# Project-MONAI/MONAI

Measured on AMD Instinct MI355X. Metric: voxels/s sliding-window 3D seg (512^3 vol, 96^3 win, ov 0.5) at 1/8 GPU, higher is better.
Workload: dtype f32; 1 GPU; BasicUNet 5-class seed 1, 512^3 CT phantom in HBM, 96^3 win ov 0.5 gaussian, sw_batch 4 (engine: <= 64 windows per launch); parallelism=1 GPU

## Files before the change

### monai_amd/csrc/kernels/conv3d_wino_h2.h

```cpp
#pragma once
#include "common.h"
#include "conv3d_h2.h"

namespace mh {

constexpr int HWG_BY = 4, HWG_BX = 16;
constexpr int HWG_RY = HWG_BY + 2, HWG_RX = HWG_BX + 2;
constexpr int HWG_NP = HWG_RY * HWG_RX;
constexpr int HWG_PB = 144;
constexpr int HWG_DB = (HWG_NP + 1) * HWG_PB;
constexpr int HWG_ZB = 32 * 1024;
constexpr int HWG_OPS = 24;
constexpr int HWG_CIN = 32, HWG_CN = 32;
constexpr int HWG_WAVES = 8;
constexpr unsigned HWG_DROP = 0x80000000u;

__device__ __forceinline__ void hw_split4(const f32x4 v, u32x2& hi, u32x2& lo) {
    _Float16 h_[4], l_[4];
#pragma unroll
    for (int i = 0; i < 4; ++i) {
        h_[i] = (_Float16)v[i];
        float r = v[i] - (float)h_[i];
        MH_OPAQUE(r);
        l_[i] = (_Float16)r;
    }
    const f16x2 h01 = {h_[0], h_[1]}, h23 = {h_[2], h_[3]}, l01 = {l_[0], l_[1]}, l23 = {l_[2], l_[3]};
    hi = u32x2{__builtin_bit_cast(unsigned, h01), __builtin_bit_cast(unsigned, h23)};
    lo = u32x2{__builtin_bit_cast(unsigned, l01), __builtin_bit_cast(unsigned, l23)};
}

__device__ __forceinline__ f32x4 hw_fma4(const f32x4 a, const float s, const f32x4 c) { return __builtin_elementwise_fma(a, f32x4{s, s, s, s}, c); }
__device__ __forceinline__ void hw_split4p(const f32x4 v, const float m1, u32x2& hi, u32x2& lo) {
#ifdef MH_SIMT_EMULATOR
    f16x2 h01, l01, h23, l23;
    h2_split_pair(v[0], v[1], m1, h01, l01);
    h2_split_pair(v[2], v[3], m1, h23, l23);
    hi = u32x2{__builtin_bit_cast(unsigned, h01), __builtin_bit_cast(unsigned, h23)};
    lo = u32x2{__builtin_bit_cast(unsigned, l01), __builtin_bit_cast(unsigned, l23)};
#else
    unsigned h0, h1, l0, l1;
    asm("v_cvt_pk_f16_f32 %0, %1, %2" : "=v"(h0) : "v"(v[0]), "v"(v[1]));
    asm("v_cvt_pk_f16_f32 %0, %1, %2" : "=v"(h1) : "v"(v[2]), "v"(v[3]));
    asm("v_fma_mixlo_f16 %0, %1, %2, %3 op_sel_hi:[1,0,0]" : "=v"(l0) : "v"(h0), "v"(m1), "v"(v[0]));
    asm("v_fma_mixlo_f16 %0, %1, %2, %3 op_sel_hi:[1,0,0]" : "=v"(l1) : "v"(h1), "v"(m1), "v"(v[2]));
    asm("v_fma_mixhi_f16 %0, %1, %2, %3 op_sel:[1,0,0] op_sel_hi:[1,0,0]" : "+v"(l0) : "v"(h0), "v"(m1), "v"(v[1]));
    asm("v_fma_mixhi_f16 %0, %1, %2, %3 op_sel:[1,0,0] op_sel_hi:[1,0,0]" : "+v"(l1) : "v"(h1), "v"(m1), "v"(v[3]));
    hi = u32x2{h0, h1};
    lo = u32x2{l0, l1};
#endif
}
__device__ __forceinline__ float hw_xchg32(const float x, const int hi) {
#ifdef MH_SIMT_EMULATOR
    (void)hi;
    return __shfl_xor(x, 32);
#else
    const auto r = __builtin_amdgcn_permlane32_swap(__builtin_bit_cast(unsigned, x), __builtin_bit_cast(unsigned, x), false, false);
    return __builtin_bit_cast(float, hi ? r[0] : r[1]);
#endif
}
#ifdef MH_SIMT_EMULATOR
#define MH_HW_KEEP_BRANCH ((void)0)
#else
#define MH_HW_KEEP_BRANCH asm volatile("" ::: "memory")
#endif

struct HwFinish {
    int co_l, fa, g4, frp, fq;
};
__device__ __forceinline__ HwFinish hw_finish_role(const int wave, const int lane) {
    HwFinish r;
    r.fq = lane & 3;
    r.frp = r.fq & 1;
    r.fa = lane >> 5;
    r.g4 = ((wave >> 1) & 1) ? (r.fq >> 1 ? 2 : 1) : (r.fq >> 1 ? 3 : 0);
    r.co_l = (wave >> 2) * 16 + (wave & 1) * 8 + ((lane >> 2) & 7);
    return r;
}

template <bool STATS, bool ACC = false, bool POOL = false>
__global__ void __launch_bounds__(512)
conv3d_k3_h2w_kernel(Tensor in, const uint4* __restrict__ wp, const float* __restrict__ wtail, const float* __restrict__ bias, Tensor out,
                     float* __restrict__ stats, int bxn, int byn, int zchunk, unsigned nblk, float* __restrict__ pmax, float* __restrict__ pmin,
                     long long pool_n_stride) {
    __shared__ __attribute__((aligned(16))) char smem[3 * HWG_DB + 2 * HWG_ZB];
    __shared__ unsigned bound_s[4];
    char* const ds = smem;
    char* const zs_ = smem + 3 * HWG_DB;
    const int tid = threadIdx.x, lane = tid & 63;
    const int wave = __builtin_amdgcn_readfirstlane(tid >> 6);
    const int wi = wave & 3, jp = wave >> 2;
    const int Cout = out.C, D = out.D, H = out.H, W = out.W;
    const long long HW = (long long)H * W, DHW = (long long)D * HW;

    const unsigned ncg = (unsigned)(Cout / HWG_CN);
    unsigned lid = xcd_remap(blockIdx.x, gridDim.x);
    const int cg = (int)(lid % ncg);
    lid /= ncg;
    const unsigned b = lid % nblk;
    const int n = (int)(lid / nblk);
    const int x0 = (int)(b % bxn) * HWG_BX, y0 = (int)((b / bxn) % byn) * HWG_BY;
    const int zs = (int)(b / (bxn * byn)) * zchunk, ze = min(zs + zchunk, D);
    const int p_first = max(zs - 1, 0), p_last = min(ze, D - 1);

    unsigned soff;
    int loff[2];
    {
        const int pr = min(lane, 53);
        const int ly = pr / 9;
        int lx = 2 * (pr - 9 * ly);
        const int gy = y0 + ly - 1;
        int gx = x0 + lx - 1;
        if (gx < 0) { gx += 1; lx += 1; }
        if (gx + 1 >= W) { gx -= 1; lx -= 1; }
        const bool ok = lane < 54 && gy >= 0 && gy < H;
        soff = ok ? 4u * (unsigned)(gy * W + gx) : 0u;
        loff[0] = (ok ? ly * HWG_RX + lx : HWG_NP) * HWG_PB;
        loff[1] = (ok ? ly * HWG_RX + lx + 1 : HWG_NP) * HWG_PB;
    }
    for (int i = tid; i < (3 * HWG_DB + 2 * HWG_ZB) / 16; i += 512) reinterpret_cast<uint4*>(smem)[i] = make_uint4(0u, 0u, 0u, 0u);
    f32x4 nra, nrb, nrs;
    {
        unsigned mb = 0u;
        if (lane < HWG_CIN) {
            const float4 a = *reinterpret_cast<const float4*>(in.nrm + (long long)n * in.nrm_n_stride + 4LL * lane);
            const unsigned bb = abs_bits(a.w);
            mb = bb == 0u ? 0x7fc00000u : bb;
        }
        mb = wave_umax(mb);
        if (tid == 0) bound_s[0] = mb;
    }
    __syncthreads();
    int e_in = 0;
    bool poisoned = false;
    {
        const unsigned mb = bound_s[0];
        poisoned = mb >= 0x7f800000u;
        e_in = poisoned ? 0 : min(max(13 - ((int)(mb >> 23) - 126), -100), 100);
        const float p_ = __uint_as_float((unsigned)(e_in + 127) << 23);
#pragma unroll
        for (int i = 0; i < 4; ++i) {
            const float4 a = *reinterpret_cast<const float4*>(in.nrm + (long long)n * in.nrm_n_stride + 4LL * (4 * wave + i));
            nra[i] = a.x * p_; nrb[i] = a.y * p_; nrs[i] = a.z;
        }
    }
    f32x4 nrk;
#pragma unroll
    for (int i = 0; i < 4; ++i) nrk[i] = nrs[i] <= 1.0f ? __builtin_inff() : -__builtin_inff();
    const auto xrs = __builtin_amdgcn_make_buffer_rsrc(const_cast<float*>(in.data + (long long)n * in.n_stride + (long long)(4 * wave) * DHW), 0, 0x7fffffff, 0x00020000);
    const unsigned hw4 = (unsigned)(HW * 4);
    unsigned voff = soff + (unsigned)p_first * hw4;
    const unsigned cso1 = (unsigned)(DHW * 4), cso2 = 2u * cso1, cso3 = 3u * cso1;
    f32x2 xin[4];
#define MH_HW_LDX                                                                                     \
    {                                                                                                 \
        xin[0] = __builtin_bit_cast(f32x2, __builtin_amdgcn_raw_buffer_load_b64(xrs, voff, 0u, 0));   \
        xin[1] = __builtin_bit_cast(f32x2, __builtin_amdgcn_raw_buffer_load_b64(xrs, voff, cso1, 0)); \
        xin[2] = __builtin_bit_cast(f32x2, __builtin_amdgcn_raw_buffer_load_b64(xrs, voff, cso2, 0)); \
        xin[3] = __builtin_bit_cast(f32x2, __builtin_amdgcn_raw_buffer_load_b64(xrs, voff, cso3, 0)); \
    }
#define MH_HW_CONV(DBO)                                                                               \
    {                                                                                                 \
        char* const db_ = ds + (DBO) + 16 * wave;                                                     \
        _Pragma("unroll") for (int j = 0; j < 2; ++j) {                                               \
            f32x4 y_;                                                                                 \
            const f32x4 t_ = __builtin_elementwise_fma(f32x4{xin[0][j], xin[1][j], xin[2][j], xin[3][j]}, nra, nrb), u_ = t_ * nrs; \
            _Pragma("unroll") for (int i = 0; i < 4; ++i) y_[i] = __builtin_amdgcn_fmed3f(t_[i], u_[i], nrk[i]);       \
            *reinterpret_cast<f32x4*>(db_ + loff[j]) = y_;                                            \
        }                                                                                             \
    }
    int staged = p_first;
#define MH_HW_ADV { voff += staged < p_last ? hw4 : 0u; staged += 1; }

    u32x4 wu[HWG_OPS];
    {
        const u32x4* wg = reinterpret_cast<const u32x4*>(wp) + ((long long)(cg * 8 + wave) * HWG_OPS) * 64 + lane;
#pragma unroll
        for (int r = 0; r < HWG_OPS; ++r) wu[r] = wg[r * 64];
    }
#define MH_HW_U(SL, T, CB, PC) __builtin_bit_cast(f16x8, wu[(((SL) * 3 + (T)) * 2 + (CB)) * 2 + (PC)])

    const int rho = lane & 15, kg = lane >> 4;
    const int tty = (rho >= 4 && rho < 12) ? 1 : 0, ttx = rho < 4 ? rho : rho < 12 ? rho - 4 : rho - 8;
    const int ra = wi == 0 ? 0 : wi == 2 ? 2 : 1, rb = wi == 0 ? 2 : wi == 1 ? 2 : wi == 2 ? 1 : 3;
    const float sgn = wi == 1 ? 1.0f : -1.0f;
    const float fsg = jp ? -1.0f : 1.0f;
    const float m1 = h2_minus_one();
    const int ab0 = ((2 * tty + ra) * HWG_RX + 2 * ttx + jp) * HWG_PB + kg * 16;
    const int ab1 = ((2 * tty + rb) * HWG_RX + 2 * ttx + jp) * HWG_PB + kg * 16;

    f32x4 acc[3][2][2];
#pragma unroll
    for (int s = 0; s < 3; ++s)
#pragma unroll
        for (int j = 0; j < 2; ++j)
#pragma unroll
            for (int c = 0; c < 2; ++c) acc[s][j][c] = f32x4{0.0f, 0.0f, 0.0f, 0.0f};

    const HwFinish fr = hw_finish_role(wave, lane);
    const int fcb = wave >> 2, fty = (wave >> 1) & 1;
    const int fa = fr.fa, fq = fr.fq, frp = fr.frp, g4 = fr.g4;
    const int ftx = 2 * fq;
    const int c16 = fr.co_l & 15;
    const int co_l = fr.co_l, co = cg * HWG_CN + co_l;
    const float bco = bias ? bias[co] : 0.0f;
    const float fs2 = fa ? -1.0f : 1.0f;
    const int zwr = wave * 4096 + (lane ^ ((lane >> 5) * 12)) * 16;
    const int zrd = fa * 4096 + fcb * 2048 + (g4 * 16 + (c16 ^ (fq >> 1 ? 12 : 0))) * 16 + frp * 8;
    float inv_a, inv_b;
    {
        const int t_ = -((int)((__float_as_uint(wtail[1]) >> 23) & 0xffu) - 127) - e_in;
        const int t1_ = t_ / 2, t2_ = t_ - t1_;
        inv_a = poisoned ? __uint_as_float(0x7fc00000u) : __uint_as_float((unsigned)(t1_ + 127) << 23);
        inv_b = __uint_as_float((unsigned)(t2_ + 127) << 23);
    }
    const auto orsrc = __builtin_amdgcn_make_buffer_rsrc(out.data + (long long)n * out.n_stride + (long long)(cg * HWG_CN) * DHW, 0, (int)(HWG_CN * DHW * 4), 0x00020000);
    const unsigned ooff = 4u * (unsigned)((long long)co_l * DHW + (long long)(y0 + 2 * fty + fa) * W + x0 + 2 * ftx);
    float pivot = 0.0f;
    bool have_c = false;
    f32x4 s1 = {0.0f, 0.0f, 0.0f, 0.0f}, s2 = s1;
    const long long PHW = (long long)(H / 2) * (W / 2), PDHW = (long long)(D / 2) * PHW;
    const auto prs = __builtin_amdgcn_make_buffer_rsrc(POOL ? (fa ? pmin : pmax) + (long long)n * pool_n_stride + (long long)(cg * HWG_CN) * PDHW : out.data, 0, POOL ? (int)(HWG_CN * PDHW * 4) : 0, 0x00020000);
    const unsigned poff = 4u * (unsigned)((long long)co_l * PDHW + (long long)((y0 >> 1) + fty) * (W / 2) + (x0 >> 1) + ftx);
    const float pk_ = fa ? -__builtin_inff() : __builtin_inff();
    f32x2 hm = {0.0f, 0.0f};
    f32x4 pv = {0.0f, 0.0f, 0.0f, 0.0f};

    u32x4 ah[2], al[2];
#define MH_HW_XFORM(DBO)                                                                              \
    {                                                                                                 \
        const char* const db_ = ds + (DBO);                                                           \
        _Pragma("unroll") for (int h = 0; h < 2; ++h) {                                               \
            f32x4 r_[3];                                                                              \
            _Pragma("unroll") for (int bq = 0; bq < 3; ++bq) {                                        \
                const f32x4 u_ = *reinterpret_cast<const f32x4*>(db_ + ab0 + bq * HWG_PB + h * 64);   \
                const f32x4 v_ = *reinterpret_cast<const f32x4*>(db_ + ab1 + bq * HWG_PB + h * 64);   \
                r_[bq] = hw_fma4(v_, sgn, u_);                                                        \
            }                                                                                         \
            const f32x4 e_ = hw_fma4(r_[2], m1, r_[0]);                                               \
            f32x4 f_;                                                                                 \
            if (jp) { f_ = hw_fma4(r_[0], m1, r_[1]); MH_HW_KEEP_BRANCH; } else f_ = r_[1] + r_[2];   \
            u32x2 hh_, ll_;                                                                           \
            hw_split4p(e_, m1, hh_, ll_); ah[0][2 * h] = hh_[0]; ah[0][2 * h + 1] = hh_[1]; al[0][2 * h] = ll_[0]; al[0][2 * h + 1] = ll_[1]; \
            hw_split4p(f_, m1, hh_, ll_); ah[1][2 * h] = hh_[0]; ah[1][2 * h + 1] = hh_[1]; al[1][2 * h] = ll_[0]; al[1][2 * h + 1] = ll_[1]; \
        }                                                                                             \
    }
#define MH_HW_MM(S, SL, CB, A, B, FRESH)                                                              \
    acc[S][SL][CB] = __builtin_amdgcn_mfma_f32_16x16x32_f16(__builtin_bit_cast(f16x8, A), B, (FRESH) ? f32x4{0.0f, 0.0f, 0.0f, 0.0f} : acc[S][SL][CB], 0, 0, 0);
#define MH_HW_MMS(S0, S1, S2)                                                                         \
    _Pragma("unroll") for (int sl = 0; sl < 2; ++sl)                                                  \
        _Pragma("unroll") for (int cb = 0; cb < 2; ++cb) {                                            \
            MH_HW_MM(S0, sl, cb, ah[sl], MH_HW_U(sl, 0, cb, 0), true)  MH_HW_MM(S1, sl, cb, ah[sl], MH_HW_U(sl, 1, cb, 0), false) MH_HW_MM(S2, sl, cb, ah[sl], MH_HW_U(sl, 2, cb, 0), false) \
            MH_HW_MM(S0, sl, cb, al[sl], MH_HW_U(sl, 0, cb, 0), false) MH_HW_MM(S1, sl, cb, al[sl], MH_HW_U(sl, 1, cb, 0), false) MH_HW_MM(S2, sl, cb, al[sl], MH_HW_U(sl, 2, cb, 0), false) \
            MH_HW_MM(S0, sl, cb, ah[sl], MH_HW_U(sl, 0, cb, 1), false) MH_HW_MM(S1, sl, cb, ah[sl], MH_HW_U(sl, 1, cb, 1), false) MH_HW_MM(S2, sl, cb, ah[sl], MH_HW_U(sl, 2, cb, 1), false) \
        }
#define MH_HW_SKIP(S0)                                                                                \
    { _Pragma("unroll") for (int sl = 0; sl < 2; ++sl) _Pragma("unroll") for (int cb = 0; cb < 2; ++cb) acc[S0][sl][cb] = f32x4{0.0f, 0.0f, 0.0f, 0.0f}; }
#define MH_HW_ZOUT(S2, Q)                                                                             \
    {                                                                                                 \
        char* const zb_ = zs_ + ((Q) & 1) * HWG_ZB + zwr;                                             \
        _Pragma("unroll") for (int cb = 0; cb < 2; ++cb) {                                            \
            *reinterpret_cast<f32x4*>(zb_ + cb * 2048) = acc[S2][0][cb] + acc[S2][1][cb];             \
            *reinterpret_cast<f32x4*>(zb_ + cb * 2048 + 1024) = acc[S2][1][cb];                       \
        }                                                                                             \
    }
#define MH_HW_FINISH(Q, ON)                                                                           \
    {                                                                                                 \
        const bool on_ = (ON);                                                                        \
        const char* const zb_ = zs_ + ((Q) & 1) * HWG_ZB + zrd;                                       \
        f32x2 z0_[3], z1_[3];                                                                         \
        _Pragma("unroll") for (int i = 0; i < 3; ++i) {                                               \
            z0_[i] = *reinterpret_cast<const f32x2*>(zb_ + i * 4096) + *reinterpret_cast<const f32x2*>(zb_ + i * 4096 + 16384 + 1024);        \
            z1_[i] = *reinterpret_cast<const f32x2*>(zb_ + i * 4096 + 1024) - *reinterpret_cast<const f32x2*>(zb_ + i * 4096 + 16384);        \
        }                                                                                             \
        const f32x2 fs_ = {fs2, fs2};                                                                 \
        const f32x2 y0_ = __builtin_elementwise_fma(z0_[2], fs_, __builtin_elementwise_fma(z0_[1], fs_, z0_[0])) * inv_a; \
        const f32x2 y1_ = __builtin_elementwise_fma(z1_[2], fs_, __builtin_elementwise_fma(z1_[1], fs_, z1_[0])) * inv_a; \
        f32x4 o_ = {__builtin_fmaf(y0_[0], inv_b, bco), __builtin_fmaf(y1_[0], inv_b, bco), __builtin_fmaf(y0_[1], inv_b, bco), __builtin_fmaf(y1_[1], inv_b, bco)}; \
        if (ACC) o_ += pv;       \
        __builtin_amdgcn_raw_buffer_store_b128(__builtin_bit_cast(u32x4, o_), orsrc, on_ ? ooff + (unsigned)(Q) * (unsigned)(HW * 4) : HWG_DROP, 0, 0); \
        if (STATS) {         \
            pivot = (on_ && !have_c) ? o_[0] : pivot;                                                 \
            have_c = have_c || on_;                                                                   \
            const f32x4 d_ = o_ - pivot, dw_ = d_ * (on_ ? 1.0f : 0.0f);                              \
            s1 += dw_;                                                                                \
            s2 = __builtin_elementwise_fma(dw_, d_, s2);                                              \
        }                                                                                             \
        if (POOL && !(HWX_OFF & 32)) {          \
            const f32x2 mx_ = {fmaxf(o_[0], o_[1]), fmaxf(o_[2], o_[3])}, mn_ = {fminf(o_[0], o_[1]), fminf(o_[2], o_[3])}; \
            const f32x2 own_ = fa ? mn_ : mx_, snd_ = fa ? mx_ : mn_;                                 \
            const f32x2 rcv_ = {hw_xchg32(snd_[0], fa), hw_xchg32(snd_[1], fa)};                      \
            const f32x2 y_ = {__builtin_amdgcn_fmed3f(own_[0], rcv_[0], pk_), __builtin_amdgcn_fmed3f(own_[1], rcv_[1], pk_)};       \
            const f32x2 f_ = {__builtin_amdgcn_fmed3f(y_[0], hm[0], pk_), __builtin_amdgcn_fmed3f(y_[1], hm[1], pk_)}; \
            const unsigned po_ = (on_ && ((Q) & 1) && !(HWX_OFF & 64)) ? poff + (unsigned)((Q) >> 1) * (unsigned)(PHW * 4) : HWG_DROP; \
            __builtin_amdgcn_raw_buffer_store_b64(__builtin_bit_cast(u32x2, f_), prs, po_, 0, 0);     \
            hm = on_ ? y_ : hm;                                                                       \
        }                                                                                             \
    }
#ifdef HWX_PROF
#define MH_HW_T(K) { const long long t_ = __builtin_readcyclecounter(); tacc[K] += t_ - tlast; tlast = t_; }
    long long tacc[8] = {0, 0, 0, 0, 0, 0, 0, 0}, tlast = __builtin_readcyclecounter();
#else
#define MH_HW_T(K)
#endif
#ifndef HWX_OFF
#define HWX_OFF 0
#endif
#ifndef HWX_DEAL
#define HWX_DEAL 2
#endif
#define MH_HW_DEAL                                                                                    \
    if constexpr (ACC || POOL) {                                                                      \
        _Pragma("unroll") for (int g_ = 0; g_ < 36; ++g_) {                                           \
            __builtin_amdgcn_sched_group_barrier(0x008, 1, 0);                                        \
            __builtin_amdgcn_sched_group_barrier(0x100, 1, 0);                                        \
            __builtin_amdgcn_sched_group_barrier(0x006, HWX_DEAL, 0);                                 \
            __builtin_amdgcn_sched_group_barrier(0x230, 1, 0);                                        \
        }                                                                                             \
    }
#define MH_HW_ITER(P, R)                                                                              \
    {                                                                                                 \
        constexpr int S0 = (3 - (R)) % 3, S1 = (S0 + 1) % 3, S2 = (S0 + 2) % 3;       \
        constexpr int db0 = (R) * HWG_DB, db2 = (((R) + 2) % 3) * HWG_DB;             \
        const int p_ = (P);                                                                           \
        const bool valid_ = p_ >= p_first && p_ <= p_last;                                            \
        const int qf_ = p_ - 2;                                                                       \
        if (ACC) { const bool nx_ = qf_ >= zs && qf_ < ze; pv = __builtin_bit_cast(f32x4, __builtin_amdgcn_raw_buffer_load_b128(orsrc, nx_ ? ooff + (unsigned)qf_ * hw4 : HWG_DROP, 0, 0)); } \
        if (valid_) { if (!(HWX_OFF & 1)) MH_HW_XFORM(db0) }                                          \
        MH_HW_T(0)                                                                                    \
        __syncthreads();                                                                              \
        MH_HW_T(1)                                                                                    \
        if (valid_) {                                                                                 \
            __builtin_amdgcn_sched_barrier(0);                                                        \
            if (!(HWX_OFF & 2)) { MH_HW_CONV(db2) MH_HW_LDX MH_HW_ADV }                               \
            if (!(HWX_OFF & 4)) MH_HW_FINISH(qf_, qf_ >= zs && qf_ < ze)                              \
            if (!(HWX_OFF & 8)) MH_HW_MMS(S0, S1, S2)                                                 \
            MH_HW_DEAL                                                                                \
            __builtin_amdgcn_sched_barrier(0);                                                        \
        } else {                                                                                      \
            MH_HW_SKIP(S0)                                                                            \
            if (!(HWX_OFF & 4)) MH_HW_FINISH(qf_, qf_ >= zs && qf_ < ze)                              \
        }                                                                                             \
        if (!(HWX_OFF & 16)) if (p_ - 1 >= zs && p_ - 1 < ze) MH_HW_ZOUT(S2, p_ - 1)                  \
        MH_HW_T(2)                                                                                    \
        __syncthreads();                                                                              \
        MH_HW_T(3)                                                                                    \
    }

    {
        const int k0 = p_first - (zs - 1);
        MH_HW_LDX MH_HW_ADV
        __syncthreads();
        MH_HW_CONV((k0 % 3) * HWG_DB)
        MH_HW_LDX MH_HW_ADV
        MH_HW_CONV(((k0 + 1) % 3) * HWG_DB)
        MH_HW_LDX MH_HW_ADV
        __syncthreads();
    }
    if (jp) __syncthreads();
    for (int p = zs - 1; p <= ze + 1; p += 3) {
        MH_HW_ITER(p, 0)
        MH_HW_ITER(p + 1, 1)
        MH_HW_ITER(p + 2, 2)
    }
    if (!jp) __syncthreads();
#ifdef HWX_PROF
    if (blockIdx.x == 0 && lane == 0) { _Pragma("unroll") for (int k = 0; k < 8; ++k) reinterpret_cast<long long*>(pmax)[wave * 8 + k] = tacc[k]; }
#endif
#undef MH_HW_T
#undef MH_HW_DEAL
#undef MH_HW_ITER
#undef MH_HW_FINISH
#undef MH_HW_ZOUT
#undef MH_HW_SKIP
#undef MH_HW_MMS
#undef MH_HW_MM
#undef MH_HW_XFORM
#undef MH_HW_U
#undef MH_HW_ADV
#undef MH_HW_CONV
#undef MH_HW_LDX

    if (STATS) {
        Stat run;
        {
            const float a1 = (s1[0] + s1[1]) + (s1[2] + s1[3]), a2 = (s2[0] + s2[1]) + (s2[2] + s2[3]);
            run.n = 4.0f * (float)(ze - zs);
            const float dm = a1 / run.n;
            run.mean = pivot + dm;
            run.m2 = fmaxf(a2 - a1 * dm, 0.0f);
        }
        __syncthreads();
        float* red = reinterpret_cast<float*>(smem);
        {
            int t_ = tid;
            MH_OPAQUE(t_);
            const HwFinish e = hw_finish_role(t_ >> 6, t_ & 63);
            float* leaf = red + (((e.co_l * 2 + e.fa) * 4 + e.g4) * 2 + e.frp) * 3;
            leaf[0] = run.n; leaf[1] = run.mean; leaf[2] = run.m2;
        }
        __syncthreads();
        if (tid < HWG_CN) {
            const auto leaf_of = [&](int a, int g, int rp) {
                const float* l = red + (((tid * 2 + a) * 4 + g) * 2 + rp) * 3;
                Stat s;
                s.n = l[0]; s.mean = l[1]; s.m2 = l[2];
                return s;
            };
            Stat st;
            st.n = 0.0f; st.mean = 0.0f; st.m2 = 0.0f;
#pragma unroll
            for (int w = 0; w < 4; ++w) {
                const int rp = w >> 1, ge = 2 * (w & 1);
                const Stat r0 = stat_merge(leaf_of(0, ge, rp), leaf_of(0, ge + 1, rp)), r1 = stat_merge(leaf_of(1, ge, rp), leaf_of(1, ge + 1, rp));
                st = stat_merge(st, stat_merge(r0, r1));
            }
            float* rec = stats + (((long long)n * Cout + cg * HWG_CN + tid) * nblk + b) * 3;
            rec[0] = st.n; rec[1] = st.mean; rec[2] = st.m2;
        }
    }
}

__global__ void conv3d_k3_h2w_scale_fix_kernel(float* __restrict__ tail) {
    if (threadIdx.x == 0 && blockIdx.x == 0) { tail[0] *= 4.0f; tail[1] *= 0.25f; }
}
__global__ void __launch_bounds__(256)
conv3d_k3_h2w_pack_kernel(const float* __restrict__ w, int Cin, int Cout, _Float16* __restrict__ packed, const float* __restrict__ tail) {
    const int idx = blockIdx.x * 256 + threadIdx.x;
    if (idx >= Cin * Cout) return;
    const int ci = idx % Cin, co = idx / Cin;
    const float s = tail[1];
    const double G[4][3] = {{1.0, 0.0, 0.0}, {0.5, 0.5, 0.5}, {0.5, -0.5, 0.5}, {0.0, 0.0, 1.0}};
    const int cg = co / HWG_CN, cb = (co % HWG_CN) / 16, nn = co % 16;
    const int kg = ci < 16 ? ci / 4 : (ci - 16) / 4, e = ci < 16 ? ci % 4 : 4 + (ci - 16) % 4;
    const int ln = kg * 16 + nn;
    for (int t = 0; t < 3; ++t) {
        double g[3][3], tm[4][3];
        for (int ky = 0; ky < 3; ++ky)
            for (int kx = 0; kx < 3; ++kx) g[ky][kx] = (double)w[((long long)co * Cin + ci) * 27 + t * 9 + ky * 3 + kx];
        for (int i = 0; i < 4; ++i)
            for (int kx = 0; kx < 3; ++kx) tm[i][kx] = G[i][0] * g[0][kx] + G[i][1] * g[1][kx] + G[i][2] * g[2][kx];
        for (int i = 0; i < 4; ++i)
            for (int j = 0; j < 4; ++j) {
                const double u = tm[i][0] * G[j][0] + tm[i][1] * G[j][1] + tm[i][2] * G[j][2];
                _Float16 pc[2];
                h2_split((float)(u * (double)s), pc[0], pc[1]);
                const int jpq = j >> 1, slot = (j == 0 || j == 3) ? 0 : 1;
                for (int p = 0; p < 2; ++p) {
                    const long long r = (((long long)(cg * 8 + jpq * 4 + i) * HWG_OPS) + ((slot * 3 + t) * 2 + cb) * 2 + p) * 64 + ln;
                    packed[r * 8 + e] = pc[p];
                }
            }
    }
}

}
```

Measured before the change: 216.3 million voxels/s.

## Peel steady-state depth loop to drop per-iteration bounds checks in Winograd conv

```diff
diff --git a/monai_amd/csrc/kernels/conv3d_wino_h2.h b/monai_amd/csrc/kernels/conv3d_wino_h2.h
--- a/monai_amd/csrc/kernels/conv3d_wino_h2.h
+++ b/monai_amd/csrc/kernels/conv3d_wino_h2.h
@@ -49,13 +49,23 @@
     lo = u32x2{l0, l1};
 #endif
 }
-__device__ __forceinline__ float hw_xchg32(const float x, const int hi) {
+__device__ __forceinline__ float hw_uniform(const float x) {
 #ifdef MH_SIMT_EMULATOR
+    return x;
+#else
+    return __builtin_bit_cast(float, __builtin_amdgcn_readfirstlane(__builtin_bit_cast(int, x)));
+#endif
+}
+__device__ __forceinline__ void hw_xchg32_pair(const float mx, const float mn, const int hi, float& own, float& rcv) {
+#ifdef MH_SIMT_EMULATOR
+    own = hi ? mn : mx;
+    rcv = __shfl_xor(hi ? mx : mn, 32);
+#else
     (void)hi;
-    return __shfl_xor(x, 32);
-#else
-    const auto r = __builtin_amdgcn_permlane32_swap(__builtin_bit_cast(unsigned, x), __builtin_bit_cast(unsigned, x), false, false);
-    return __builtin_bit_cast(float, hi ? r[0] : r[1]);
+    const auto r = __builtin_amdgcn_permlane32_swap(__builtin_bit_cast(unsigned, mx), __builtin_bit_cast(unsigned, mn), false, false);
+    const unsigned r0 = r[0], r1 = r[1];
+    own = __builtin_bit_cast(float, r0);
+    rcv = __builtin_bit_cast(float, r1);
 #endif
 }
 #ifdef MH_SIMT_EMULATOR
@@ -140,12 +150,12 @@
 #pragma unroll
         for (int i = 0; i < 4; ++i) {
             const float4 a = *reinterpret_cast<const float4*>(in.nrm + (long long)n * in.nrm_n_stride + 4LL * (4 * wave + i));
-            nra[i] = a.x * p_; nrb[i] = a.y * p_; nrs[i] = a.z;
+            nra[i] = hw_uniform(a.x * p_); nrb[i] = a.y * p_; nrs[i] = a.z;
         }
     }
     f32x4 nrk;
 #pragma unroll
-    for (int i = 0; i < 4; ++i) nrk[i] = nrs[i] <= 1.0f ? __builtin_inff() : -__builtin_inff();
+    for (int i = 0; i < 4; ++i) nrk[i] = hw_uniform(nrs[i] <= 1.0f ? __builtin_inff() : -__builtin_inff());
     const auto xrs = __builtin_amdgcn_make_buffer_rsrc(const_cast<float*>(in.data + (long long)n * in.n_stride + (long long)(4 * wave) * DHW), 0, 0x7fffffff, 0x00020000);
     const unsigned hw4 = (unsigned)(HW * 4);
     unsigned voff = soff + (unsigned)p_first * hw4;
@@ -161,12 +171,12 @@
 #define MH_HW_CONV(DBO)                                                                               \
     {                                                                                                 \
         char* const db_ = ds + (DBO) + 16 * wave;                                                     \
-        _Pragma("unroll") for (int j = 0; j < 2; ++j) {                                               \
-            f32x4 y_;                                                                                 \
-            const f32x4 t_ = __builtin_elementwise_fma(f32x4{xin[0][j], xin[1][j], xin[2][j], xin[3][j]}, nra, nrb), u_ = t_ * nrs; \
-            _Pragma("unroll") for (int i = 0; i < 4; ++i) y_[i] = __builtin_amdgcn_fmed3f(t_[i], u_[i], nrk[i]);       \
-            *reinterpret_cast<f32x4*>(db_ + loff[j]) = y_;                                            \
-        }                                                                                             \
+        f32x4 y_[2];                                                                                  \
+        _Pragma("unroll") for (int i = 0; i < 4; ++i) {                                               \
+            const f32x2 t_ = __builtin_elementwise_fma(xin[i], f32x2{nra[i], nra[i]}, f32x2{nrb[i], nrb[i]}), u_ = t_ * nrs[i]; \
+            _Pragma("unroll") for (int j = 0; j < 2; ++j) y_[j][i] = __builtin_amdgcn_fmed3f(t_[j], u_[j], nrk[i]);       \
+        }                                                                                             \
+        _Pragma("unroll") for (int j = 0; j < 2; ++j) *reinterpret_cast<f32x4*>(db_ + loff[j]) = y_[j]; \
     }
     int staged = p_first;
 #define MH_HW_ADV { voff += staged < p_last ? hw4 : 0u; staged += 1; }
@@ -210,8 +220,8 @@
     {
         const int t_ = -((int)((__float_as_uint(wtail[1]) >> 23) & 0xffu) - 127) - e_in;
         const int t1_ = t_ / 2, t2_ = t_ - t1_;
-        inv_a = poisoned ? __uint_as_float(0x7fc00000u) : __uint_as_float((unsigned)(t1_ + 127) << 23);
-        inv_b = __uint_as_float((unsigned)(t2_ + 127) << 23);
+        inv_a = hw_uniform(poisoned ? __uint_as_float(0x7fc00000u) : __uint_as_float((unsigned)(t1_ + 127) << 23));
+        inv_b = hw_uniform(__uint_as_float((unsigned)(t2_ + 127) << 23));
     }
     const auto orsrc = __builtin_amdgcn_make_buffer_rsrc(out.data + (long long)n * out.n_stride + (long long)(cg * HWG_CN) * DHW, 0, (int)(HWG_CN * DHW * 4), 0x00020000);
     const unsigned ooff = 4u * (unsigned)((long long)co_l * DHW + (long long)(y0 + 2 * fty + fa) * W + x0 + 2 * ftx);
@@ -219,8 +229,11 @@
     bool have_c = false;
     f32x4 s1 = {0.0f, 0.0f, 0.0f, 0.0f}, s2 = s1;
     const long long PHW = (long long)(H / 2) * (W / 2), PDHW = (long long)(D / 2) * PHW;
-    const auto prs = __builtin_amdgcn_make_buffer_rsrc(POOL ? (fa ? pmin : pmax) + (long long)n * pool_n_stride + (long long)(cg * HWG_CN) * PDHW : out.data, 0, POOL ? (int)(HWG_CN * PDHW * 4) : 0, 0x00020000);
-    const unsigned poff = 4u * (unsigned)((long long)co_l * PDHW + (long long)((y0 >> 1) + fty) * (W / 2) + (x0 >> 1) + ftx);
+    float* const pbase_mx = POOL ? pmax + (long long)n * pool_n_stride + (long long)(cg * HWG_CN) * PDHW : out.data;
+    float* const pbase_mn = POOL ? pmin + (long long)n * pool_n_stride + (long long)(cg * HWG_CN) * PDHW : out.data;
+    const int pbytes = POOL ? (int)(HWG_CN * PDHW * 4) : 0;
+    const unsigned phw4 = (unsigned)(PHW * 4);
+    const unsigned poff = (4u * (unsigned)((long long)co_l * PDHW + (long long)((y0 >> 1) + fty) * (W / 2) + (x0 >> 1) + ftx)) | (fa ? HWG_DROP : 0u);
     const float pk_ = fa ? -__builtin_inff() : __builtin_inff();
     f32x2 hm = {0.0f, 0.0f};
     f32x4 pv = {0.0f, 0.0f, 0.0f, 0.0f};
@@ -263,9 +276,9 @@
             *reinterpret_cast<f32x4*>(zb_ + cb * 2048 + 1024) = acc[S2][1][cb];                       \
         }                                                                                             \
     }
-#define MH_HW_FINISH(Q, ON)                                                                           \
-    {                                                                                                 \
-        const bool on_ = (ON);                                                                        \
+#define MH_HW_FINISH(Q, ON, ST)                                                                       \
+    {                                                                                                 \
+        const bool on_ = (ST) ? true : (ON);                                                          \
         const char* const zb_ = zs_ + ((Q) & 1) * HWG_ZB + zrd;                                       \
         f32x2 z0_[3], z1_[3];                                                                         \
         _Pragma("unroll") for (int i = 0; i < 3; ++i) {                                               \
@@ -277,22 +290,28 @@
         const f32x2 y1_ = __builtin_elementwise_fma(z1_[2], fs_, __builtin_elementwise_fma(z1_[1], fs_, z1_[0])) * inv_a; \
         f32x4 o_ = {__builtin_fmaf(y0_[0], inv_b, bco), __builtin_fmaf(y1_[0], inv_b, bco), __builtin_fmaf(y0_[1], inv_b, bco), __builtin_fmaf(y1_[1], inv_b, bco)}; \
         if (ACC) o_ += pv;       \
-        __builtin_amdgcn_raw_buffer_store_b128(__builtin_bit_cast(u32x4, o_), orsrc, on_ ? ooff + (unsigned)(Q) * (unsigned)(HW * 4) : HWG_DROP, 0, 0); \
+        if (ST) __builtin_amdgcn_raw_buffer_store_b128(__builtin_bit_cast(u32x4, o_), orsrc, ooff, (unsigned)(Q) * hw4, 0); \
+        else __builtin_amdgcn_raw_buffer_store_b128(__builtin_bit_cast(u32x4, o_), orsrc, on_ ? ooff + (unsigned)(Q) * hw4 : HWG_DROP, 0, 0); \
         if (STATS) {         \
-            pivot = (on_ && !have_c) ? o_[0] : pivot;                                                 \
-            have_c = have_c || on_;                                                                   \
-            const f32x4 d_ = o_ - pivot, dw_ = d_ * (on_ ? 1.0f : 0.0f);                              \
+            if (!(ST)) {                                                                              \
+                pivot = (on_ && !have_c) ? o_[0] : pivot;                                             \
+                have_c = have_c || on_;                                                               \
+            }                                                                                         \
+            const f32x4 d_ = o_ - pivot, dw_ = (ST) ? d_ : d_ * (on_ ? 1.0f : 0.0f);                  \
             s1 += dw_;                                                                                \
             s2 = __builtin_elementwise_fma(dw_, d_, s2);                                              \
         }                                                                                             \
         if (POOL && !(HWX_OFF & 32)) {          \
             const f32x2 mx_ = {fmaxf(o_[0], o_[1]), fmaxf(o_[2], o_[3])}, mn_ = {fminf(o_[0], o_[1]), fminf(o_[2], o_[3])}; \
-            const f32x2 own_ = fa ? mn_ : mx_, snd_ = fa ? mx_ : mn_;                                 \
-            const f32x2 rcv_ = {hw_xchg32(snd_[0], fa), hw_xchg32(snd_[1], fa)};                      \
-            const f32x2 y_ = {__builtin_amdgcn_fmed3f(own_[0], rcv_[0], pk_), __builtin_amdgcn_fmed3f(own_[1], rcv_[1], pk_)};       \
+            float own0_, rcv0_, own1_, rcv1_;                                                         \
+            hw_xchg32_pair(mx_[0], mn_[0], fa, own0_, rcv0_);                                         \
+            hw_xchg32_pair(mx_[1], mn_[1], fa, own1_, rcv1_);                                         \
+            const f32x2 y_ = {__builtin_amdgcn_fmed3f(own0_, rcv0_, pk_), __builtin_amdgcn_fmed3f(own1_, rcv1_, pk_)};       \
             const f32x2 f_ = {__builtin_amdgcn_fmed3f(y_[0], hm[0], pk_), __builtin_amdgcn_fmed3f(y_[1], hm[1], pk_)}; \
-            const unsigned po_ = (on_ && ((Q) & 1) && !(HWX_OFF & 64)) ? poff + (unsigned)((Q) >> 1) * (unsigned)(PHW * 4) : HWG_DROP; \
-            __builtin_amdgcn_raw_buffer_store_b64(__builtin_bit_cast(u32x2, f_), prs, po_, 0, 0);     \
+            const int pn_ = (on_ && ((Q) & 1) && !(HWX_OFF & 64)) ? pbytes : 0;                       \
+            const unsigned ps_ = (unsigned)((Q) >> 1) * phw4;                                         \
+            __builtin_amdgcn_raw_buffer_store_b64(__builtin_bit_cast(u32x2, f_), __builtin_amdgcn_make_buffer_rsrc(pbase_mx, 0, pn_, 0x00020000), poff, ps_, 0); \
+            __builtin_amdgcn_raw_buffer_store_b64(__builtin_bit_cast(u32x2, f_), __builtin_amdgcn_make_buffer_rsrc(pbase_mn, 0, pn_, 0x00020000), poff ^ HWG_DROP, ps_, 0); \
             hm = on_ ? y_ : hm;                                                                       \
         }                                                                                             \
     }
@@ -317,14 +336,17 @@
             __builtin_amdgcn_sched_group_barrier(0x230, 1, 0);                                        \
         }                                                                                             \
     }
-#define MH_HW_ITER(P, R)                                                                              \
+#define MH_HW_ITER(P, R, ST)                                                                          \
     {                                                                                                 \
         constexpr int S0 = (3 - (R)) % 3, S1 = (S0 + 1) % 3, S2 = (S0 + 2) % 3;       \
         constexpr int db0 = (R) * HWG_DB, db2 = (((R) + 2) % 3) * HWG_DB;             \
         const int p_ = (P);                                                                           \
-        const bool valid_ = p_ >= p_first && p_ <= p_last;                                            \
+        const bool valid_ = (ST) ? true : (p_ >= p_first && p_ <= p_last);                            \
         const int qf_ = p_ - 2;                                                                       \
-        if (ACC) { const bool nx_ = qf_ >= zs && qf_ < ze; pv = __builtin_bit_cast(f32x4, __builtin_amdgcn_raw_buffer_load_b128(orsrc, nx_ ? ooff + (unsigned)qf_ * hw4 : HWG_DROP, 0, 0)); } \
+        if (ACC) {                                                                                    \
+            if (ST) pv = __builtin_bit_cast(f32x4, __builtin_amdgcn_raw_buffer_load_b128(orsrc, ooff, (unsigned)qf_ * hw4, 0)); \
+            else { const bool nx_ = qf_ >= zs && qf_ < ze; pv = __builtin_bit_cast(f32x4, __builtin_amdgcn_raw_buffer_load_b128(orsrc, nx_ ? ooff + (unsigned)qf_ * hw4 : HWG_DROP, 0, 0)); } \
+        }                                                                                             \
         if (valid_) { if (!(HWX_OFF & 1)) MH_HW_XFORM(db0) }                                          \
         MH_HW_T(0)                                                                                    \
         __syncthreads();                                                                              \
@@ -332,15 +354,15 @@
         if (valid_) {                                                                                 \
             __builtin_amdgcn_sched_barrier(0);                                                        \
             if (!(HWX_OFF & 2)) { MH_HW_CONV(db2) MH_HW_LDX MH_HW_ADV }                               \
-            if (!(HWX_OFF & 4)) MH_HW_FINISH(qf_, qf_ >= zs && qf_ < ze)                              \
+            if (!(HWX_OFF & 4)) MH_HW_FINISH(qf_, qf_ >= zs && qf_ < ze, ST)                          \
             if (!(HWX_OFF & 8)) MH_HW_MMS(S0, S1, S2)                                                 \
             MH_HW_DEAL                                                                                \
             __builtin_amdgcn_sched_barrier(0);                                                        \
         } else {                                                                                      \
             MH_HW_SKIP(S0)                                                                            \
-            if (!(HWX_OFF & 4)) MH_HW_FINISH(qf_, qf_ >= zs && qf_ < ze)                              \
-        }                                                                                             \
-        if (!(HWX_OFF & 16)) if (p_ - 1 >= zs && p_ - 1 < ze) MH_HW_ZOUT(S2, p_ - 1)                  \
+            if (!(HWX_OFF & 4)) MH_HW_FINISH(qf_, qf_ >= zs && qf_ < ze, false)                       \
+        }                                                                                             \
+        if (!(HWX_OFF & 16)) if ((ST) || (p_ - 1 >= zs && p_ - 1 < ze)) MH_HW_ZOUT(S2, p_ - 1)        \
         MH_HW_T(2)                                                                                    \
         __syncthreads();                                                                              \
         MH_HW_T(3)                                                                                    \
@@ -357,11 +379,14 @@
         __syncthreads();
     }
     if (jp) __syncthreads();
-    for (int p = zs - 1; p <= ze + 1; p += 3) {
-        MH_HW_ITER(p, 0)
-        MH_HW_ITER(p + 1, 1)
-        MH_HW_ITER(p + 2, 2)
-    }
+    int p = zs - 1;
+#define MH_HW_STEADY(P) ((P) >= zs + 5 && (P) + 2 <= p_last && (P) + 1 < ze)
+#define MH_HW_BLOCK(ST) { MH_HW_ITER(p, 0, ST) MH_HW_ITER(p + 1, 1, ST) MH_HW_ITER(p + 2, 2, ST) }
+    for (; p <= ze + 1 && !MH_HW_STEADY(p); p += 3) MH_HW_BLOCK(false)
+    for (; MH_HW_STEADY(p); p += 3) MH_HW_BLOCK(true)
+    for (; p <= ze + 1; p += 3) MH_HW_BLOCK(false)
+#undef MH_HW_BLOCK
+#undef MH_HW_STEADY
     if (!jp) __syncthreads();
 #ifdef HWX_PROF
     if (blockIdx.x == 0 && lane == 0) { _Pragma("unroll") for (int k = 0; k < 8; ++k) reinterpret_cast<long long*>(pmax)[wave * 8 + k] = tacc[k]; }
```

After: 220.8 million voxels/s (median of 6 runs). 1.02x the previous value.
